# statgen/popscle

Measured on AMD Instinct MI355X. Metric: cell-sample-pair LLs/sec (singlet+doublet), demuxlet 10k cells×16 samples, higher is better.
Workload: dtype f64; 1 GPU; demuxlet synthetic PLP (BASELINE.json configs[1]): 10000 cells x 16 samples x 50000 SNPs per GPU, alpha grid [0.0, 0.5], 9537271 entries, 12399525 reads; cells_per_gpu=10000, samples=16, snps=50000, entries_per_gpu=9537271, lls_per_cell=256, parallelism=cells sharded x1

## Files before the change

### popscle_amd/csrc/demux_oct.hip

```cpp
#include <algorithm>
#include <vector>

#include <rocprim/device/device_radix_sort.hpp>

#include "demux_call_body.hpp"

namespace {

constexpr int O_NLUT = 129;
constexpr int O_LPAD = 3;

template <int P>
struct og {
  static_assert(P == 8 || P == 16, "eight or sixteen lanes per entry");
  static constexpr int SLOTS = 64 / P;
  static constexpr int BATCH = P;
  static constexpr int NROT = P / 2 - 1;
  static constexpr int N_ACC = 3 + 4 * NROT + 3;
  static constexpr int N_HYP = N_ACC * P;
  static constexpr int SLOT_STRIDE = 9 * P + 2;
  static constexpr int ACC_AB = 2;
  static constexpr int ACC_F_AB = 3 + 4 * NROT, ACC_F_AA = ACC_F_AB + 1, ACC_F_BB = ACC_F_AB + 2;
  __host__ __device__ static constexpr int acc_single(int c) { return c; }
  __host__ __device__ static constexpr int acc_rot(int t, int c, int d) { return 3 + (t - 1) * 4 + c * 2 + d; }
  __host__ __device__ static constexpr int ror(int t) { return 0x120 + (P == 8 ? 2 * t : t); }
  __device__ static __forceinline__ int pos(int lane) { return P == 8 ? (lane >> 1) & 7 : lane & 15; }
  __device__ static __forceinline__ int slot(int lane) { return P == 8 ? ((lane >> 4) << 1) | (lane & 1) : lane >> 4; }
  __device__ static __forceinline__ int lane0(int lane) { return P == 8 ? lane & ~14 : lane & ~15; }
  static constexpr uint32_t MROW = 32u * P;
  static constexpr int TROW = 6 * P;
};

template <int CTRL>
__device__ __forceinline__ double dpp_rot(double x) {
  int lo = __double2loint(x), hi = __double2hiint(x);
  lo = __builtin_amdgcn_mov_dpp(lo, CTRL, 0xF, 0xF, false);
  hi = __builtin_amdgcn_mov_dpp(hi, CTRL, 0xF, 0xF, false);
  return __hiloint2double(hi, lo);
}

template <int P>
__global__ void oct_pmap_kernel(int32_t* pmap) {
  const int lane = threadIdx.x;
  const int p = og<P>::pos(lane);
  wave_for<1, P / 2 + 1>([&](auto tc) {
    constexpr int t = decltype(tc)::value;
    const int pt = __builtin_amdgcn_mov_dpp(p, og<P>::ror(t), 0xF, 0xF, false);
    if (og<P>::slot(lane) == 0) pmap[(t - 1) * P + p] = pt;
  });
}

__global__ void __launch_bounds__(64)
    oct_partition_kernel(int n_chunks, const row_chunk* __restrict__ chunks, const quad_entry* __restrict__ qent,
                         const uint32_t* __restrict__ lin, const uint8_t* __restrict__ reads,
                         const double* __restrict__ gp0s, quad_entry* __restrict__ out, quad_lrec* __restrict__ lrec,
                         int32_t* __restrict__ nlin) {
  const int q = blockIdx.x * blockDim.x + threadIdx.x;
  if (q >= n_chunks) return;
  const int64_t e0 = chunks[q].e0;
  const int len = chunks[q].len;
  int w = 0;
  for (int i = 0; i < len; ++i) {
    const int64_t e = e0 + i;
    if ((lin[e >> 5] >> (e & 31)) & 1u) {
      const quad_entry p = qent[e];
      uint32_t code = MUXGL_READ_OTHER;
      for (uint32_t k = 0; k < p.nreads; ++k) {
        const uint32_t bb = k < 4 ? (p.first4 >> (8 * k)) & 0xffu : (uint32_t)reads[(int64_t)p.r0 + k];
        if (bb != MUXGL_READ_OTHER) code = bb;
      }
      if (gp0s[p.snp] < 0.0) code = MUXGL_READ_OTHER;
      lrec[e0 + w] = quad_lrec{p.snp, code};
      out[e0 + w++] = p;
    }
  }
  nlin[q] = w;
  for (int i = 0; i < len; ++i) {
    const int64_t e = e0 + i;
    if (!((lin[e >> 5] >> (e & 31)) & 1u)) out[e0 + w++] = qent[e];
  }
}

constexpr int QUAD_BUCKET = 1024;
__global__ void __launch_bounds__(256)
    quad_order_key_kernel(int n_chunks, int bucket, const row_chunk* __restrict__ chunks,
                          const int32_t* __restrict__ chunk_nlin, uint64_t* __restrict__ key, int32_t* __restrict__ iota) {
  const int w = blockIdx.x * blockDim.x + threadIdx.x;
  if (w >= n_chunks) return;
  const int nl = chunk_nlin[w], len = chunks[w].len;
  const uint64_t bg = (uint64_t)min(len - nl, 1023), bl = (uint64_t)min(nl, 1023);
  key[w] = ((uint64_t)(w / bucket) << 40) | ((1023u - bg) << 30) | ((1023u - bl) << 20) | (uint64_t)(w % bucket);
  iota[w] = w;
}

__global__ void __launch_bounds__(256)
    oct_unit_steps_kernel(int n_units, int n_chunks, int slots, const int32_t* __restrict__ order,
                          const int32_t* __restrict__ nlin, int32_t* __restrict__ steps) {
  const int u = blockIdx.x * blockDim.x + threadIdx.x;
  if (u >= n_units) return;
  int m = 0;
  for (int k = 0; k < slots; ++k) {
    const int w = u * slots + k;
    if (w < n_chunks) m = max(m, nlin[order[w]]);
  }
  steps[u] = m > 0 ? (m + 2) / 3 * 3 + O_LPAD : 0;
}

__global__ void __launch_bounds__(256)
    oct_repack_kernel(int n_units, int n_chunks, const row_chunk* __restrict__ chunks, const int32_t* __restrict__ order,
                      const int32_t* __restrict__ nlin, const quad_lrec* __restrict__ lrec,
                      const int32_t* __restrict__ steps, const int64_t* __restrict__ unit_ptr, uint32_t S_dummy,
                      int slots, uint32_t mrow , uint2* __restrict__ orec) {
  const int t = blockIdx.x * blockDim.x + threadIdx.x;
  const int u = t / slots, slot = t % slots;
  if (u >= n_units) return;
  const int w = u * slots + slot;
  int64_t e0 = 0;
  int nl = 0;
  if (w < n_chunks) {
    const int q = order[w];
    e0 = chunks[q].e0;
    nl = nlin[q];
  }
  uint2* dst = orec + unit_ptr[u] + slot;
  const int n = steps[u];
  for (int i = 0; i < n; ++i) {
    uint2 r{S_dummy * mrow, (uint32_t)(O_NLUT - 1) * 32u};
    if (i < nl) {
      const quad_lrec x = lrec[e0 + i];
      const uint32_t idx = x.code == MUXGL_READ_OTHER ? (uint32_t)(O_NLUT - 1) : ((x.code >> 7) << 6) | (x.code & 0x3fu);
      r = uint2{(uint32_t)x.snp * mrow, idx * 32u};
    }
    dst[(size_t)i * slots] = r;
  }
}

template <int P, bool UNIT_S>
#ifndef OCT_WAVES
#define OCT_WAVES 3
#endif
__global__ void __launch_bounds__(64, P == 8 ? OCT_WAVES : 2)
    demux_oct_kernel(const row_chunk* __restrict__ chunks, int n_chunks, const quad_entry* __restrict__ qent,
                     const uint2* __restrict__ orec, const int64_t* __restrict__ unit_ptr,
                     const int32_t* __restrict__ chunk_nlin,
                     const int32_t* __restrict__ order, const uint8_t* __restrict__ reads,
                     const double* __restrict__ gpo, const double* __restrict__ gmo,
                     const double* __restrict__ gp0s, int32_t S_dummy, const double* __restrict__ lut_g,
                     const int32_t* __restrict__ chunk_pos, double* __restrict__ part_m, int32_t* __restrict__ part_e) {
  __shared__ double lut[384];
  __shared__ __align__(16) double ablut[O_NLUT * 4];
  using G = og<P>;
  constexpr int ON_ACC = G::N_ACC, O_SLOTS = G::SLOTS, O_BATCH = G::BATCH, O_SLOT_STRIDE = G::SLOT_STRIDE;
  constexpr int O_ACC_AB = G::ACC_AB, O_ACC_F_AB = G::ACC_F_AB, O_ACC_F_AA = G::ACC_F_AA, O_ACC_F_BB = G::ACC_F_BB;
  __shared__ __align__(16) double pgs[O_SLOTS * O_SLOT_STRIDE];
  __shared__ int32_t snps[64], snps_nx[64];

  const int lane = threadIdx.x;
  const int p = G::pos(lane);
  const int slot = G::slot(lane);
  for (int i = lane; i < 384; i += 64) lut[i] = lut_g[i];
  for (int i = lane; i < O_NLUT; i += 64) {
    const uint32_t bq = (uint32_t)i & 0x3f;
    const bool ref = (i >> 6) == 0;
    const double e3 = lut_g[256 + bq], mt = lut_g[128 + bq];
    const double pR = ref ? mt : e3, pA = ref ? e3 : mt;
    const double mx = fmax(pR, pA);
    double x = __builtin_amdgcn_rcp(mx);
    x = fma(x, fma(-mx, x, 1.0), x);
    x = fma(x, fma(-mx, x, 1.0), x);
    const double cc = 1.0 / (1.0 + 1e-10);
    const double sc = cc * x, tt = 1e-10 * cc;
    const bool none = i == O_NLUT - 1;
    const double B = none ? 0.0 : (pA - pR) * (0.25 * sc);
    ablut[4 * i] = none ? 1.0 : fma(pR, sc, tt);
    ablut[4 * i + 1] = B;
    ablut[4 * i + 2] = B + B;
    ablut[4 * i + 3] = 0.0;
  }
  __syncthreads();

  const int unit = xcd_swizzle(blockIdx.x, gridDim.x >> 3);
  const int wq = unit * O_SLOTS + slot;
  const uint32_t p16 = (uint32_t)p * 16u;
  const int q = wq < n_chunks ? (order ? order[wq] : wq) : n_chunks;
  int64_t e0 = 0;
  int len = 0;
  int32_t qpos = 0;
  if (q < n_chunks) {
    e0 = chunks[q].e0;
    len = chunks[q].len;
    qpos = chunk_pos[q];
  }
  const int nl = (chunk_nlin && q < n_chunks) ? chunk_nlin[q] : 0;
  const int nLmax = wave_max_i32(nl);
  const int ngmax = wave_max_i32(len - nl);
  const int nb = (ngmax + O_BATCH - 1) / O_BATCH;

  double acc[ON_ACC];
  int32_t exs[ON_ACC];
#pragma unroll
  for (int a = 0; a < ON_ACC; ++a) {
    acc[a] = 1.0;
    exs[a] = 0;
  }
  double accW[2] = {1.0, 1.0};
  int32_t exW[2] = {0, 0};
  double accH = 1.0;
  int32_t exH = 0;

  auto renorm = [&]() __attribute__((always_inline)) {
#pragma unroll
    for (int a = 0; a < ON_ACC; ++a) prodacc_renorm(acc[a], exs[a]);
    prodacc_renorm(accW[0], exW[0]);
    prodacc_renorm(accW[1], exW[1]);
    prodacc_renorm(accH, exH);
  };

  if (nLmax > 0) {
    struct rowl_t {
      double sa, ra, sb, rb;
    };
    auto load_rowl = [&](rowl_t& R, uint32_t row_off) __attribute__((always_inline)) {
      if (UNIT_S) {
        const double2 v = *reinterpret_cast<const double2*>(reinterpret_cast<const char*>(gmo) + (size_t)((row_off >> 1) + p16));
        R.sa = R.sb = 1.0;
        R.ra = v.x;
        R.rb = v.y;
        return;
      }
      const double2* pc = reinterpret_cast<const double2*>(reinterpret_cast<const char*>(gmo) + (size_t)(row_off + p16));
      const double2 va = pc[0], vb = pc[P];
      R.sa = va.x;
      R.ra = va.y;
      R.sb = vb.x;
      R.rb = vb.y;
    };
    const uint2* lr = orec + unit_ptr[unit] + slot;
    struct ab_t {
      double A, B, B2;
    };
    auto ab_of = [&](const uint2& rc) __attribute__((always_inline)) {
      const double* t = reinterpret_cast<const double*>(reinterpret_cast<const char*>(ablut) + rc.y);
      const double2 v = *reinterpret_cast<const double2*>(t);
      return ab_t{v.x, v.y, t[2]};
    };
    auto sweepL = [&](const rowl_t& R, const ab_t& ab) __attribute__((always_inline)) {
      const double A = ab.A, B = ab.B, B2 = ab.B2;
      if (!UNIT_S) {
        accW[0] *= R.sa;
        accW[1] *= R.sb;
      }
      acc[G::acc_single(0)] *= fma(B2, R.ra, A);
      acc[G::acc_single(1)] *= fma(B2, R.rb, A);
      const double Xa = fma(B, R.ra, A), Xb = fma(B, R.rb, A);
      acc[O_ACC_AB] *= fma(B, R.rb, Xa);
      wave_for<1, G::NROT + 1>([&](auto tc) {
        constexpr int t = decltype(tc)::value;
        const double Pa = dpp_rot<G::ror(t)>(R.ra), Pb = dpp_rot<G::ror(t)>(R.rb);
        acc[G::acc_rot(t, 0, 0)] *= fma(B, Pa, Xa);
        acc[G::acc_rot(t, 0, 1)] *= fma(B, Pb, Xa);
        acc[G::acc_rot(t, 1, 0)] *= fma(B, Pa, Xb);
        acc[G::acc_rot(t, 1, 1)] *= fma(B, Pb, Xb);
      });
      {
        const double Pa = dpp_rot<G::ror(P / 2)>(R.ra), Pb = dpp_rot<G::ror(P / 2)>(R.rb);
        acc[O_ACC_F_AB] *= fma(B, Pb, Xa);
        acc[O_ACC_F_AA] *= fma(B, Pa, Xa);
        acc[O_ACC_F_BB] *= fma(B, Pb, Xb);
      }
    };
    auto step = [&](int i, const rowl_t& Rc, rowl_t& Rnn, const ab_t& abc, ab_t& abn, uint2& rc0, const uint2& rc1,
                    const uint2& rc2) __attribute__((always_inline)) {
      rc0 = lr[(i + 3) * O_SLOTS];
      abn = ab_of(rc1);
      load_rowl(Rnn, rc2.x);
      __builtin_amdgcn_sched_barrier(0);
      sweepL(Rc, abc);
      __builtin_amdgcn_sched_barrier(0);
    };
    rowl_t L0, L1, L2;
    ab_t ab0, ab1, ab2;
    uint2 ra = lr[0], rb = lr[O_SLOTS], rc = lr[2 * O_SLOTS];
    load_rowl(L0, ra.x);
    load_rowl(L1, rb.x);
    ab0 = ab_of(ra);
    int since = 0;
    for (int i = 0; i < nLmax; i += 3) {
      step(i, L0, L2, ab0, ab1, ra, rb, rc);
      step(i + 1, L1, L0, ab1, ab2, rb, rc, ra);
      step(i + 2, L2, L1, ab2, ab0, rc, ra, rb);
      if (++since == 10) {
        since = 0;
        renorm();
      }
    }
    renorm();
  }

  if (nb > 0) {
    const int last = len > 0 ? len - 1 : 0;
    auto fetch_meta = [&](int b) __attribute__((always_inline)) {
      const int idx = nl + b * O_BATCH + p;
      return qent[e0 + (idx < last ? idx : last)];
    };
    auto snp_of = [&](const quad_entry& r, int b) __attribute__((always_inline)) { return (nl + b * O_BATCH + p < len) ? r.snp : -1; };
    quad_entry precA = fetch_meta(0), precB = fetch_meta(1);
    double hs_cur = gp0s[precA.snp];

    struct row_t {
      double a[3], b[3];
    };
    auto load_row = [&](row_t& R, int32_t s) __attribute__((always_inline)) {
      const double2* pc = reinterpret_cast<const double2*>(gpo + (size_t)s * G::TROW) + p;
      const double2 v0 = pc[0], v1 = pc[P], v2 = pc[2 * P];
      R.a[0] = v0.x;
      R.a[1] = v0.y;
      R.a[2] = v1.x;
      R.b[0] = v1.y;
      R.b[1] = v2.x;
      R.b[2] = v2.y;
    };

    auto phase1 = [&](int b) __attribute__((always_inline)) {
      const int32_t sa = snp_of(precA, b);
      const int32_t s = (hs_cur >= 0.0) ? sa : -1;
      const double hs_out = (s >= 0) ? hs_cur : 1.0;
      const int64_t r0 = precA.r0, r1 = (int64_t)precA.r0 + precA.nreads;
      const uint32_t first4 = precA.first4;
      precA = precB;
      precB = fetch_meta(b + 2);
      hs_cur = gp0s[precA.snp];
      double q0[3], q1[5];
      {
        double pRk[4], pAk[4];
        const uint32_t nr = (s >= 0) ? (uint32_t)(r1 - r0) : 0u;
#pragma unroll
        for (int k = 0; k < 4; ++k) {
          const uint32_t bb = (first4 >> (8 * k)) & 0xffu;
          const uint32_t bq = bb & 0x7f;
          const double e3 = lut[256 + bq], mt = lut[128 + bq];
          const bool use = (uint32_t)k < nr && bb != MUXGL_READ_OTHER;
          const bool ref = (bb >> 7) == 0;
          pRk[k] = use ? (ref ? mt : e3) : 1.0;
          pAk[k] = use ? (ref ? e3 : mt) : 1.0;
        }
        {
          const double d = pAk[0] - pRk[0];
          const double mid = fma(d, 0.5, pRk[0]);
          q0[0] = pRk[0];
          q0[1] = mid;
          q0[2] = pAk[0];
          q1[0] = pRk[0];
          q1[1] = fma(d, 0.25, pRk[0]);
          q1[2] = mid;
          q1[3] = fma(d, 0.75, pRk[0]);
          q1[4] = pAk[0];
        }
#pragma unroll
        for (int k = 1; k < 4; ++k) {
          const double d = pAk[k] - pRk[k];
          const double mid = fma(d, 0.5, pRk[k]);
          q0[0] *= pRk[k];
          q0[1] *= mid;
          q0[2] *= pAk[k];
          q1[0] *= pRk[k];
          q1[1] *= fma(d, 0.25, pRk[k]);
          q1[2] *= mid;
          q1[3] *= fma(d, 0.75, pRk[k]);
          q1[4] *= pAk[k];
        }
        if (nr > 4) {
          int since = 4;
          for (int64_t rr = r0 + 4; rr < r1; ++rr) {
            const uint32_t bb = (uint32_t)reads[rr];
            if (bb == MUXGL_READ_OTHER) continue;
            const uint32_t al = bb >> 7, bq = bb & 0x7f;
            const double e3 = lut[256 + bq], mt = lut[128 + bq];
            const double pR = (al == 0) ? mt : e3, pA = (al == 0) ? e3 : mt;
            const double d = pA - pR;
            const double mid = fma(d, 0.5, pR);
            q0[0] *= pR;
            q0[1] *= mid;
            q0[2] *= pA;
            q1[0] *= pR;
            q1[1] *= fma(d, 0.25, pR);
            q1[2] *= mid;
            q1[3] *= fma(d, 0.75, pR);
            q1[4] *= pA;
            if (++since >= 32) {
              since = 0;
              double mx = fmax(fmax(q0[0], q0[1]), q0[2]);
#pragma unroll
              for (int t = 0; t < 5; ++t) mx = fmax(mx, q1[t]);
              const double inv = 1.0 / mx;
#pragma unroll
              for (int l = 0; l < 3; ++l) q0[l] *= inv;
#pragma unroll
              for (int t = 0; t < 5; ++t) q1[t] *= inv;
            }
          }
        }
        double mx = fmax(fmax(q0[0], q0[1]), q0[2]);
#pragma unroll
        for (int t = 0; t < 5; ++t) mx = fmax(mx, q1[t]);
        double x = __builtin_amdgcn_rcp(mx);
        x = fma(x, fma(-mx, x, 1.0), x);
        x = fma(x, fma(-mx, x, 1.0), x);
        const double cc = 1.0 / (1.0 + 1e-10);
        const double sc = (s >= 0) ? cc * x : 1.0, tt = (s >= 0) ? 1e-10 * cc : 0.0;
#pragma unroll
        for (int l = 0; l < 3; ++l) q0[l] = fma(q0[l], sc, tt);
#pragma unroll
        for (int t = 0; t < 5; ++t) q1[t] = fma(q1[t], sc, tt);
      }
      double* dst = pgs + slot * O_SLOT_STRIDE + p * 8;
      dst[0] = q0[0];
      dst[1] = q0[1];
      dst[2] = q0[2];
#pragma unroll
      for (int t = 0; t < 5; ++t) dst[3 + t] = q1[t];
      pgs[slot * O_SLOT_STRIDE + 8 * P + p] = hs_out;
      snps[slot * P + p] = (s >= 0) ? s : S_dummy;
      const int32_t sn = snp_of(precA, b + 1);
      snps_nx[slot * P + p] = (sn >= 0) ? sn : S_dummy;
    };

    auto sweep_entry = [&](const row_t& R, int i) __attribute__((always_inline)) {
      const double* qq = pgs + slot * O_SLOT_STRIDE + i * 8;
      const double a0 = qq[0], a1 = qq[1], a2 = qq[2];
      const double b0 = qq[3], b1 = qq[4], b2 = qq[5], b3 = qq[6], b4 = qq[7];
      if (!UNIT_S) accH *= pgs[slot * O_SLOT_STRIDE + 8 * P + i];
      acc[G::acc_single(0)] *= fma(R.a[2], a2, fma(R.a[1], a1, R.a[0] * a0));
      acc[G::acc_single(1)] *= fma(R.b[2], a2, fma(R.b[1], a1, R.b[0] * a0));
      double ua[3], ub[3];
      ua[0] = fma(R.a[2], b2, fma(R.a[1], b1, R.a[0] * b0));
      ua[1] = fma(R.a[2], b3, fma(R.a[1], b2, R.a[0] * b1));
      ua[2] = fma(R.a[2], b4, fma(R.a[1], b3, R.a[0] * b2));
      ub[0] = fma(R.b[2], b2, fma(R.b[1], b1, R.b[0] * b0));
      ub[1] = fma(R.b[2], b3, fma(R.b[1], b2, R.b[0] * b1));
      ub[2] = fma(R.b[2], b4, fma(R.b[1], b3, R.b[0] * b2));
      auto dot = [](const double* g, const double* u) { return fma(g[2], u[2], fma(g[1], u[1], g[0] * u[0])); };
      acc[O_ACC_AB] *= dot(R.b, ua);
      wave_for<1, G::NROT + 1>([&](auto tc) {
        constexpr int t = decltype(tc)::value;
        double Pa[3], Pb[3];
        Pa[0] = dpp_rot<G::ror(t)>(R.a[0]);
        Pa[1] = dpp_rot<G::ror(t)>(R.a[1]);
        Pa[2] = dpp_rot<G::ror(t)>(R.a[2]);
        Pb[0] = dpp_rot<G::ror(t)>(R.b[0]);
        Pb[1] = dpp_rot<G::ror(t)>(R.b[1]);
        Pb[2] = dpp_rot<G::ror(t)>(R.b[2]);
        acc[G::acc_rot(t, 0, 0)] *= dot(Pa, ua);
        acc[G::acc_rot(t, 0, 1)] *= dot(Pb, ua);
        acc[G::acc_rot(t, 1, 0)] *= dot(Pa, ub);
        acc[G::acc_rot(t, 1, 1)] *= dot(Pb, ub);
      });
      {
        constexpr int CF = G::ror(P / 2);
        double Pa[3], Pb[3];
        Pa[0] = dpp_rot<CF>(R.a[0]);
        Pa[1] = dpp_rot<CF>(R.a[1]);
        Pa[2] = dpp_rot<CF>(R.a[2]);
        Pb[0] = dpp_rot<CF>(R.b[0]);
        Pb[1] = dpp_rot<CF>(R.b[1]);
        Pb[2] = dpp_rot<CF>(R.b[2]);
        acc[O_ACC_F_AB] *= dot(Pb, ua);
        acc[O_ACC_F_AA] *= dot(Pa, ua);
        acc[O_ACC_F_BB] *= dot(Pb, ub);
      }
    };

    auto batch = [&](int b, row_t& X, row_t& Y, row_t& Z) __attribute__((always_inline)) {
      phase1(b);
      __syncthreads();
      const int32_t* sn = snps + slot * P;
      const int32_t* sx = snps_nx + slot * P;
      const int lim = (b == nb - 1) ? ngmax - b * O_BATCH : O_BATCH;
      auto set = [&](auto ic) __attribute__((always_inline)) -> row_t& {
        constexpr int i = decltype(ic)::value % 3;
        if constexpr (i == 0) return X;
        else if constexpr (i == 1) return Y;
        else return Z;
      };
      bool go = true;
      wave_for<0, P>([&](auto ec) {
        constexpr int e = decltype(ec)::value;
        if (!go) return;
        load_row(set(std::integral_constant<int, e + 2>{}), e + 2 < P ? sn[e + 2 < P ? e + 2 : 0] : sx[e + 2 - P < 0 ? 0 : e + 2 - P]);
        __builtin_amdgcn_sched_barrier(0);
        sweep_entry(set(ec), e);
        __builtin_amdgcn_sched_barrier(0);
        if (lim <= e + 1) go = false;
      });
      if (P == 16 || (b & 1)) renorm();
      __syncthreads();
    };

    row_t R0, R1, R2;
    snps_nx[slot * P + p] = (snp_of(precA, 0) >= 0) ? precA.snp : S_dummy;
    __syncthreads();
    load_row(R0, snps_nx[slot * P + 0]);
    load_row(R1, snps_nx[slot * P + 1]);
    __syncthreads();
    for (int b = 0; b < nb; b += 3) {
      batch(b, R0, R1, R2);
      if (b + 1 >= nb) break;
      if (P == 8) batch(b + 1, R2, R0, R1);
      else batch(b + 1, R1, R2, R0);
      if (b + 2 >= nb) break;
      if (P == 8) batch(b + 2, R1, R2, R0);
      else batch(b + 2, R2, R0, R1);
    }
    renorm();
  }

  {
    int32_t exa[ON_ACC];
    const double wa = accW[0], wb = accW[1];
    const int32_t ea = exW[0], eb = exW[1];
    const int src0 = G::lane0(lane);
    const double W0 = __shfl(wa, src0, 64) * accH;
    const int32_t e0w = __shfl(ea, src0, 64) + exH;
    acc[G::acc_single(0)] *= wa * W0;
    exa[G::acc_single(0)] = ea + e0w;
    acc[G::acc_single(1)] *= wb * W0;
    exa[G::acc_single(1)] = eb + e0w;
    acc[O_ACC_AB] *= wa * wb;
    exa[O_ACC_AB] = ea + eb;
    wave_for<1, G::NROT + 1>([&](auto tc) {
      constexpr int T = decltype(tc)::value, CTRL = G::ror(T);
      const double pa = dpp_rot<CTRL>(wa), pb = dpp_rot<CTRL>(wb);
      const int32_t qa = __builtin_amdgcn_mov_dpp(ea, CTRL, 0xF, 0xF, false);
      const int32_t qb = __builtin_amdgcn_mov_dpp(eb, CTRL, 0xF, 0xF, false);
      acc[G::acc_rot(T, 0, 0)] *= wa * pa;
      exa[G::acc_rot(T, 0, 0)] = ea + qa;
      acc[G::acc_rot(T, 0, 1)] *= wa * pb;
      exa[G::acc_rot(T, 0, 1)] = ea + qb;
      acc[G::acc_rot(T, 1, 0)] *= wb * pa;
      exa[G::acc_rot(T, 1, 0)] = eb + qa;
      acc[G::acc_rot(T, 1, 1)] *= wb * pb;
      exa[G::acc_rot(T, 1, 1)] = eb + qb;
    });
    {
      constexpr int CF = G::ror(P / 2);
      const double pa = dpp_rot<CF>(wa), pb = dpp_rot<CF>(wb);
      const int32_t qa = __builtin_amdgcn_mov_dpp(ea, CF, 0xF, 0xF, false);
      const int32_t qb = __builtin_amdgcn_mov_dpp(eb, CF, 0xF, 0xF, false);
      acc[O_ACC_F_AB] *= wa * pb;
      exa[O_ACC_F_AB] = ea + qb;
      acc[O_ACC_F_AA] *= wa * pa;
      exa[O_ACC_F_AA] = ea + qa;
      acc[O_ACC_F_BB] *= wb * pb;
      exa[O_ACC_F_BB] = eb + qb;
    }
    if (q < n_chunks) {
#pragma unroll
      for (int a = 0; a < ON_ACC; ++a) {
        int e;
        const double m = frexp(acc[a], &e);
        part_m[((size_t)qpos * ON_ACC + a) * P + p] = m;
        part_e[((size_t)qpos * ON_ACC + a) * P + p] = exs[a] + e + exa[a];
      }
    }
  }
}

template <int P>
__device__ __forceinline__ bool oct_decode(int idx, const int32_t* __restrict__ pmap, int V, int& j, int& k) {
  using G = og<P>;
  const int a = idx / P, p = idx % P;
  bool publish = true;
  if (a < 2) {
    j = p + P * a;
    k = 0;
  } else if (a == G::ACC_AB) {
    j = p + P;
    k = p;
  } else if (a < G::ACC_F_AB) {
    const int t = (a - 3) >> 2, c = ((a - 3) >> 1) & 1, d = (a - 3) & 1;
    j = p + P * c;
    k = pmap[t * P + p] + P * d;
  } else {
    const int pf = pmap[G::NROT * P + p];
    if (a == G::ACC_F_AB) {
      j = p;
      k = pf + P;
    } else if (a == G::ACC_F_AA) {
      j = p;
      k = pf;
      publish = p < pf;
    } else {
      j = p + P;
      k = pf + P;
      publish = p < pf;
    }
  }
  return publish && j < V && k < V;
}

__device__ __forceinline__ double oct_log(double m, int64_t e) { return pos_log(m, (double)e); }

template <int P>
__device__ __forceinline__ bool oct_hypothesis(int idx, int64_t c0, int64_t c1, const double* __restrict__ part_m,
                                               const int32_t* __restrict__ part_e, const int32_t* __restrict__ pmap, int V,
                                               int& j, int& k, double& v) {
  constexpr int O_NHYP = og<P>::N_HYP;
  if (!oct_decode<P>(idx, pmap, V, j, k)) return false;
  double m = 1.0;
  int64_t e = 0;
  int cnt = 0;
  for (int64_t ci = c0; ci < c1; ci += 8) {
    double pm[8];
    int32_t pe[8];
#pragma unroll
    for (int u = 0; u < 8; ++u) {
      const bool ok = ci + u < c1;
      const size_t o = (size_t)(ok ? ci + u : c0) * O_NHYP + idx;
      pm[u] = ok ? part_m[o] : 1.0;
      pe[u] = ok ? part_e[o] : 0;
    }
#pragma unroll
    for (int u = 0; u < 8; ++u) {
      m *= pm[u];
      e += pe[u];
    }
    if (++cnt == 64) {
      cnt = 0;
      int ee;
      m = frexp(m, &ee);
      e += ee;
    }
  }
  v = oct_log(m, e);
  return true;
}

__global__ void __launch_bounds__(256)
    oct_chunk_pos_kernel(int64_t n_chunks, const int32_t* __restrict__ cell_chunks, int32_t* __restrict__ pos) {
  const int64_t ci = (int64_t)blockIdx.x * blockDim.x + threadIdx.x;
  if (ci < n_chunks) pos[cell_chunks[ci]] = (int32_t)ci;
}

template <int P>
__global__ void __launch_bounds__(192)
    demux_oct_reduce_kernel(const int64_t* __restrict__ cell_chunk_ptr, const double* __restrict__ part_m,
                            const int32_t* __restrict__ part_e, const int32_t* __restrict__ pmap, int V,
                            double* __restrict__ ll) {
  const int64_t c = blockIdx.x;
  const int64_t c0 = cell_chunk_ptr[c], c1 = cell_chunk_ptr[c + 1];
  if (c0 == c1) return;
  double* out = ll + (size_t)c * V * V * 2;
  for (int idx = threadIdx.x; idx < og<P>::N_HYP; idx += 192) {
    int j, k;
    double v;
    if (!oct_hypothesis<P>(idx, c0, c1, part_m, part_e, pmap, V, j, k, v)) continue;
    if (idx < 2 * P) {
      out[((size_t)j * V + k) * 2 + 0] = v;
    } else {
      out[((size_t)j * V + k) * 2 + 1] = v;
      out[((size_t)k * V + j) * 2 + 1] = v;
    }
  }
}

#ifndef QF_CELLS_N
#define QF_CELLS_N 4
#endif
template <int P>
__global__ void __launch_bounds__(256)
    demux_oct_finish_kernel(int64_t C, const int64_t* __restrict__ cell_ptr, const int64_t* __restrict__ cell_chunk_ptr,
                            const double* __restrict__ part_m, const int32_t* __restrict__ part_e,
                            const int32_t* __restrict__ pmap, int V,
                            muxgl_call::call_alpha al, double doublet_prior, muxgl_demux_cell* __restrict__ out) {
  constexpr int QF_CELLS = P == 8 ? QF_CELLS_N : 1, THREADS = 256, O_NHYP = og<P>::N_HYP;
  static_assert(P == 16 || QF_CELLS * 64 == THREADS, "a wave per cell at P = 8");
  constexpr int LD = 4 * P + 1;
  __shared__ double llt[QF_CELLS][2 * P * LD];
  __shared__ __align__(16) muxgl_demux_cell rec[QF_CELLS];
  __shared__ int64_t ccp[QF_CELLS + 1];
  static_assert(sizeof(muxgl_demux_cell) % 16 == 0, "records are copied out in 16-byte pieces");
  const int64_t cbase = (int64_t)blockIdx.x * QF_CELLS;
  const int tid = threadIdx.x;
  if (tid <= QF_CELLS) ccp[tid] = cell_chunk_ptr[cbase + tid <= C ? cbase + tid : C];
  for (int t = tid; t < QF_CELLS * 2 * P * LD; t += THREADS) (&llt[0][0])[t] = 0.0;
  __syncthreads();
  constexpr int NH = (QF_CELLS * O_NHYP + THREADS - 1) / THREADS;
  int hj[NH], hk[NH], hidx[NH], hlc[NH];
  int64_t h0[NH];
  int hn[NH];
  bool hv[NH];
  double hm[NH];
  int64_t he[NH];
  int nmax = 0;
#pragma unroll
  for (int i = 0; i < NH; ++i) {
    const int w = tid + i * THREADS;
    const int lc = w < QF_CELLS * O_NHYP ? w / O_NHYP : 0;
    hlc[i] = lc;
    hidx[i] = w - lc * O_NHYP;
    h0[i] = ccp[lc];
    hn[i] = (int)(ccp[lc + 1] - ccp[lc]);
    hv[i] = w < QF_CELLS * O_NHYP && hn[i] > 0 && oct_decode<P>(hidx[i] < O_NHYP ? hidx[i] : 0, pmap, V, hj[i], hk[i]);
    if (!hv[i]) hn[i] = 0, hidx[i] = 0;
    hm[i] = 1.0;
    he[i] = 0;
    nmax = hn[i] > nmax ? hn[i] : nmax;
  }
  int cnt = 0;
  for (int ci = 0; ci < nmax; ci += 4) {
    double pm[NH][4];
    int32_t pe[NH][4];
#pragma unroll
    for (int i = 0; i < NH; ++i)
#pragma unroll
      for (int u = 0; u < 4; ++u) {
        const bool ok = ci + u < hn[i];
        const size_t o = (ok ? (size_t)(h0[i] + ci + u) * O_NHYP : 0) + hidx[i];
        const double vm = part_m[o];
        const int32_t ve = part_e[o];
        pm[i][u] = ok ? vm : 1.0;
        pe[i][u] = ok ? ve : 0;
      }
#pragma unroll
    for (int i = 0; i < NH; ++i)
#pragma unroll
      for (int u = 0; u < 4; ++u) {
        hm[i] *= pm[i][u];
        he[i] += pe[i][u];
      }
    if (++cnt == 128) {
      cnt = 0;
#pragma unroll
      for (int i = 0; i < NH; ++i) {
        int ee;
        hm[i] = frexp(hm[i], &ee);
        he[i] += ee;
      }
    }
  }
#pragma unroll
  for (int i = 0; i < NH; ++i) {
    if (!hv[i]) continue;
    const double v = oct_log(hm[i], he[i]);
    if (hidx[i] < 2 * P) {
      llt[hlc[i]][hj[i] * LD + hk[i] * 2 + 0] = v;
    } else {
      llt[hlc[i]][hj[i] * LD + hk[i] * 2 + 1] = v;
      llt[hlc[i]][hk[i] * LD + hj[i] * 2 + 1] = v;
    }
  }
  __syncthreads();
  if constexpr (P == 8) {
    __shared__ muxgl_call::call_partial parts[QF_CELLS];
    const int lc = tid >> 6;
    const int64_t c = cbase + lc;
    const muxgl_call::call_partial cp = muxgl_call::demux_call_scan<16, 4>(tid & 63, c < C, V, 2, al, llt[lc], LD);
    if ((tid & 63) == 0) parts[lc] = cp;
    __syncthreads();
    if (tid < QF_CELLS && cbase + tid < C)
      muxgl_call::demux_call_decide(parts[tid], (int32_t)(cell_ptr[cbase + tid + 1] - cell_ptr[cbase + tid]), V, 2, al,
                                    &rec[tid]);
  } else {
    if (tid < 64)
      muxgl_call::demux_call_group<64>(tid, cbase < C, cbase < C ? (int32_t)(cell_ptr[cbase + 1] - cell_ptr[cbase]) : 0, V, 2,
                                       al, doublet_prior, llt[0], &rec[0], LD);
  }
  __syncthreads();
  constexpr int NQ = (int)(sizeof(muxgl_demux_cell) / 16);
  if (tid < QF_CELLS * NQ && cbase + tid / NQ < C)
    reinterpret_cast<uint4*>(out + cbase)[tid] = reinterpret_cast<const uint4*>(&rec[0])[tid];
}

}

int quad_launch_order(muxgl_handle* h, const row_chunk* d_chunks, const int32_t* d_nlin, int64_t n, int32_t** order) {
  int32_t* d_iota = nullptr;
  uint64_t *d_key = nullptr, *d_key2 = nullptr;
  void* d_tmp = nullptr;
  auto cleanup = [&]() {
    dev_free(&d_iota);
    dev_free(&d_key);
    dev_free(&d_key2);
    if (d_tmp) (void)hipFree(d_tmp);
    d_tmp = nullptr;
  };
  if (dev_alloc(h, order, (size_t)n) || dev_alloc(h, &d_iota, (size_t)n) || dev_alloc(h, &d_key, (size_t)n) ||
      dev_alloc(h, &d_key2, (size_t)n)) {
    cleanup();
    return 1;
  }
  int bucket = QUAD_BUCKET;
  if (const char* ev = getenv("MUXGL_QUAD_BUCKET")) bucket = atoi(ev) > 0 ? atoi(ev) : bucket;
  if (bucket > (1 << 20)) bucket = 1 << 20;
  hipLaunchKernelGGL(quad_order_key_kernel, dim3((unsigned)((n + 255) / 256)), dim3(256), 0, h->stream, (int)n, bucket, d_chunks,
                     d_nlin, d_key, d_iota);
  size_t tmp_bytes = 0;
  hipError_t e = rocprim::radix_sort_pairs(nullptr, tmp_bytes, d_key, d_key2, d_iota, *order, (size_t)n, 0u, 64u, h->stream);
  if (e == hipSuccess) e = dev_malloc_retry((void**)&d_tmp, tmp_bytes ? tmp_bytes : 1);
  if (e == hipSuccess) e = rocprim::radix_sort_pairs(d_tmp, tmp_bytes, d_key, d_key2, d_iota, *order, (size_t)n, 0u, 64u, h->stream);
  if (e == hipSuccess) e = hipStreamSynchronize(h->stream);
  cleanup();
  if (e != hipSuccess) MUXGL_FAIL(h, "quad_launch_order: %s", hipGetErrorString(e));
  return 0;
}

namespace {
template <int P>
int oct_launch_t(muxgl_handle* h, const muxgl_demux_params* p) {
  constexpr int O_SLOTS = og<P>::SLOTS, O_NHYP = og<P>::N_HYP;
  muxgl_row_state* st = h->qrow;
  if (!st->d_tmap || st->tmap_p != P) {
    if (dev_alloc(h, &st->d_tmap, (size_t)(P / 2) * P)) return 1;
    hipLaunchKernelGGL(oct_pmap_kernel<P>, dim3(1), dim3(64), 0, h->stream, st->d_tmap);
    HIPCHK(h, hipGetLastError());
    st->tmap_p = P;
  }
  const size_t need = (size_t)st->n_chunks * O_NHYP;
  if (need > st->part_cap) {
    if (dev_alloc(h, &st->d_part, need)) return 1;
    st->part_cap = need;
  }
  if (need > st->part_e_cap) {
    if (dev_alloc(h, &st->d_part_e, need)) return 1;
    st->part_e_cap = need;
  }
  if (!st->d_chunk_pos) {
    if (dev_alloc(h, &st->d_chunk_pos, (size_t)(st->n_chunks ? st->n_chunks : 1))) return 1;
    if (st->n_chunks)
      hipLaunchKernelGGL(oct_chunk_pos_kernel, dim3((unsigned)((st->n_chunks + 255) / 256)), dim3(256), 0, h->stream, st->n_chunks,
                         st->d_cell_chunks, st->d_chunk_pos);
    HIPCHK(h, hipGetLastError());
  }
  const bool use_lin = h->d_lin && h->d_gmq && !(h->flags & MUXGL_FLAG_NO_LINEAR_ENTRIES);
  const unsigned blocks = (unsigned)((((st->n_chunks + O_SLOTS - 1) / O_SLOTS) + 7) / 8 * 8);
  if (use_lin && !st->d_chunk_nlin && st->n_chunks) {
    quad_lrec* d_lrec = nullptr;
    int32_t* d_steps = nullptr;
    auto cleanup = [&]() {
      dev_free(&d_lrec);
      dev_free(&d_steps);
    };
    if (dev_alloc(h, &st->d_qent_lin, (size_t)h->nnz) || dev_alloc(h, &st->d_chunk_nlin, (size_t)st->n_chunks) ||
        dev_alloc(h, &d_lrec, (size_t)h->nnz)) {
      cleanup();
      return 1;
    }
    hipLaunchKernelGGL(oct_partition_kernel, dim3((unsigned)((st->n_chunks + 63) / 64)), dim3(64), 0, h->stream,
                       (int)st->n_chunks, st->d_chunks, h->d_qent, h->d_lin, h->d_reads, h->d_gp0s, st->d_qent_lin,
                       d_lrec, st->d_chunk_nlin);
    if (hipGetLastError() != hipSuccess || quad_launch_order(h, st->d_chunks, st->d_chunk_nlin, st->n_chunks, &st->d_quad_order)) {
      cleanup();
      MUXGL_FAIL(h, "demux_oct_launch: partition failed");
    }
    const int n_units = (int)blocks;
    std::vector<int32_t> steps((size_t)n_units);
    std::vector<int64_t> uptr((size_t)n_units + 1, 0);
    if (dev_alloc(h, &d_steps, (size_t)n_units)) {
      cleanup();
      return 1;
    }
    hipLaunchKernelGGL(oct_unit_steps_kernel, dim3((unsigned)((n_units + 255) / 256)), dim3(256), 0, h->stream, n_units,
                       (int)st->n_chunks, O_SLOTS, st->d_quad_order, st->d_chunk_nlin, d_steps);
    hipError_t e = hipMemcpyAsync(steps.data(), d_steps, sizeof(int32_t) * (size_t)n_units, hipMemcpyDeviceToHost, h->stream);
    if (e == hipSuccess) e = hipStreamSynchronize(h->stream);
    for (int u = 0; u < n_units; ++u) uptr[(size_t)u + 1] = uptr[(size_t)u] + (int64_t)steps[(size_t)u] * O_SLOTS;
    if (e != hipSuccess || dev_alloc(h, &st->d_unit_ptr, uptr.size()) || dev_alloc(h, &st->d_orec, (size_t)uptr.back() + 1)) {
      cleanup();
      MUXGL_FAIL(h, "demux_oct_launch: record tables");
    }
    e = hipMemcpyAsync(st->d_unit_ptr, uptr.data(), sizeof(int64_t) * uptr.size(), hipMemcpyHostToDevice, h->stream);
    hipLaunchKernelGGL(oct_repack_kernel, dim3((unsigned)(((size_t)n_units * O_SLOTS + 255) / 256)), dim3(256), 0, h->stream,
                       n_units, (int)st->n_chunks, st->d_chunks, st->d_quad_order, st->d_chunk_nlin, d_lrec, d_steps,
                       st->d_unit_ptr, (uint32_t)h->S, O_SLOTS, og<P>::MROW, st->d_orec);
    if (e == hipSuccess) e = hipGetLastError();
    if (e == hipSuccess) e = hipStreamSynchronize(h->stream);
    cleanup();
    if (e != hipSuccess) MUXGL_FAIL(h, "demux_oct_launch: %s", hipGetErrorString(e));
  }
  tic(h, MUXGL_T_DEMUX_SWEEP);
  if (blocks) {
    auto kern = h->gp_unit_sums ? demux_oct_kernel<P, true> : demux_oct_kernel<P, false>;
    hipLaunchKernelGGL(kern, dim3(blocks), dim3(64), 0,
                       h->stream, st->d_chunks, (int)st->n_chunks,
                       use_lin ? st->d_qent_lin : h->d_qent, st->d_orec, st->d_unit_ptr,
                       use_lin ? st->d_chunk_nlin : (const int32_t*)nullptr,
                       use_lin ? st->d_quad_order : (const int32_t*)nullptr, h->d_reads,
                       h->d_gpq, h->d_gmq, h->d_gp0s, (int32_t)h->S, h->d_lut, st->d_chunk_pos, st->d_part, st->d_part_e);
    HIPCHK(h, hipGetLastError());
  }
  toc_tic(h, MUXGL_T_DEMUX_SWEEP, MUXGL_T_DEMUX_REDUCE);
  if (h->want_full_ll) {
    hipLaunchKernelGGL(demux_oct_reduce_kernel<P>, dim3((unsigned)h->C), dim3(192), 0, h->stream, st->d_cell_chunk_ptr,
                       st->d_part, st->d_part_e, st->d_tmap, h->V, h->d_ll);
  } else {
    const muxgl_call::call_alpha al = muxgl_call::make_call_alpha(p, h->V);
    constexpr int QF_CELLS = P == 8 ? QF_CELLS_N : 1;
    hipLaunchKernelGGL(demux_oct_finish_kernel<P>, dim3((unsigned)((h->C + QF_CELLS - 1) / QF_CELLS)), dim3(256), 0,
                       h->stream, h->C, h->d_cell_ptr, st->d_cell_chunk_ptr, st->d_part, st->d_part_e, st->d_tmap, h->V, al,
                       p->doublet_prior, h->h_dcells);
    h->records_on_host = true;
  }
  HIPCHK(h, hipGetLastError());
  toc(h, MUXGL_T_DEMUX_REDUCE);
  return 0;
}
}

int demux_oct_launch(muxgl_handle* h, const muxgl_demux_params* p) {
  return h->V <= 16 ? oct_launch_t<8>(h, p) : oct_launch_t<16>(h, p);
}
```

Before: 7.647 billion LLs/s.

## Pack partial mantissa and exponent into one 8-byte word with escape side channel

The sweep kernel now stores each partial product as a single 8-byte word: 52 mantissa bits plus a biased 12-bit exponent. A separate int32 side array is written only when the value falls outside the normal range. The reduce and finish kernels read one word per partial instead of a double plus an int32, and use a precomputed slot table for hypothesis decode. The finish kernel also now gives each cell its own wave with no per-hypothesis length masking. This is meant to cut memory traffic and per-element work in the reduction, at the cost of extra bit manipulation and a rare slow escape path.

```diff
diff --git a/popscle_amd/csrc/demux_oct.hip b/popscle_amd/csrc/demux_oct.hip
--- a/popscle_amd/csrc/demux_oct.hip
+++ b/popscle_amd/csrc/demux_oct.hip
@@ -31,6 +31,25 @@
   static constexpr int TROW = 6 * P;
 };
 
+constexpr int OCT_EBIAS = 4093;
+constexpr uint32_t OCT_EFIELD_ESC = 4095u;
+__device__ __forceinline__ void oct_pack(double m, int32_t E, size_t o, uint2* __restrict__ part, int32_t* __restrict__ part_e) {
+  const uint32_t hi = (uint32_t)__double2hiint(m), lo = (uint32_t)__double2loint(m);
+  const bool plain = (hi >> 20) == 0x3FEu && (uint32_t)(E + OCT_EBIAS) < OCT_EFIELD_ESC;
+  part[o] = uint2{lo, (hi & 0xFFFFFu) | ((plain ? (uint32_t)(E + OCT_EBIAS) : OCT_EFIELD_ESC) << 20)};
+  if (!plain) part_e[o] = (int32_t)(((uint32_t)E & 0xFFFFFu) | ((hi >> 20) << 20));
+}
+__device__ __forceinline__ void oct_unpack(uint2 w, size_t o, const int32_t* __restrict__ part_e, double& m, int32_t& eb) {
+  uint32_t top = 0x3FEu;
+  eb = (int32_t)(w.y >> 20);
+  if (w.y >= (OCT_EFIELD_ESC << 20)) {
+    const int32_t pe = part_e[o];
+    top = (uint32_t)pe >> 20;
+    eb = ((int32_t)((uint32_t)pe << 12) >> 12) + OCT_EBIAS;
+  }
+  m = __hiloint2double((int)((w.y & 0xFFFFFu) | (top << 20)), (int)w.x);
+}
+
 template <int CTRL>
 __device__ __forceinline__ double dpp_rot(double x) {
   int lo = __double2loint(x), hi = __double2hiint(x);
@@ -146,7 +165,7 @@
                      const int32_t* __restrict__ order, const uint8_t* __restrict__ reads,
                      const double* __restrict__ gpo, const double* __restrict__ gmo,
                      const double* __restrict__ gp0s, int32_t S_dummy, const double* __restrict__ lut_g,
-                     const int32_t* __restrict__ chunk_pos, double* __restrict__ part_m, int32_t* __restrict__ part_e) {
+                     const int32_t* __restrict__ chunk_pos, uint2* __restrict__ part, int32_t* __restrict__ part_e) {
   __shared__ double lut[384];
   __shared__ __align__(16) double ablut[O_NLUT * 4];
   using G = og<P>;
@@ -558,15 +577,14 @@
       for (int a = 0; a < ON_ACC; ++a) {
         int e;
         const double m = frexp(acc[a], &e);
-        part_m[((size_t)qpos * ON_ACC + a) * P + p] = m;
-        part_e[((size_t)qpos * ON_ACC + a) * P + p] = exs[a] + e + exa[a];
+        oct_pack(m, exs[a] + e + exa[a], ((size_t)qpos * ON_ACC + a) * P + p, part, part_e);
       }
     }
   }
 }
 
 template <int P>
-__device__ __forceinline__ bool oct_decode(int idx, const int32_t* __restrict__ pmap, int V, int& j, int& k) {
+__device__ __forceinline__ bool oct_decode(int idx, const int32_t* __restrict__ pmap, int& j, int& k) {
   using G = og<P>;
   const int a = idx / P, p = idx % P;
   bool publish = true;
@@ -595,44 +613,80 @@
       publish = p < pf;
     }
   }
-  return publish && j < V && k < V;
-}
+  return publish;
+}
+
+template <int P>
+__global__ void __launch_bounds__(64) oct_slot_kernel(const int32_t* __restrict__ pmap, int32_t* __restrict__ slots) {
+  const int idx = blockIdx.x * blockDim.x + threadIdx.x;
+  if (idx >= og<P>::N_HYP) return;
+  int j, k;
+  const bool publish = oct_decode<P>(idx, pmap, j, k);
+  slots[idx] = j | (k << 8) | ((publish ? (j > k ? j : k) : 255) << 16);
+}
+constexpr int32_t OCT_SLOT_NONE = 255 << 16;
+__device__ __forceinline__ bool oct_slot_live(int32_t s, int V) { return ((s >> 16) & 0xff) < V; }
 
 __device__ __forceinline__ double oct_log(double m, int64_t e) { return pos_log(m, (double)e); }
 
-template <int P>
-__device__ __forceinline__ bool oct_hypothesis(int idx, int64_t c0, int64_t c1, const double* __restrict__ part_m,
-                                               const int32_t* __restrict__ part_e, const int32_t* __restrict__ pmap, int V,
-                                               int& j, int& k, double& v) {
-  constexpr int O_NHYP = og<P>::N_HYP;
-  if (!oct_decode<P>(idx, pmap, V, j, k)) return false;
-  double m = 1.0;
-  int64_t e = 0;
+template <int NH, int U, int O_NHYP, int R>
+__device__ __forceinline__ void oct_fold_trip(const uint2* __restrict__ pb, const int32_t* __restrict__ pe, int64_t ci,
+                                              const int (&off)[NH], double (&hm)[NH], int64_t (&he)[NH]) {
+  uint2 w[NH][R];
+  uint32_t top = 0;
+#pragma unroll
+  for (int i = 0; i < NH; ++i)
+#pragma unroll
+    for (int u = 0; u < R; ++u) {
+      w[i][u] = pb[(size_t)(ci + u) * O_NHYP + off[i]];
+      top = w[i][u].y > top ? w[i][u].y : top;
+    }
+  if (__builtin_expect(top < (OCT_EFIELD_ESC << 20), 1)) {
+#pragma unroll
+    for (int i = 0; i < NH; ++i) {
+      uint32_t es = 0;
+#pragma unroll
+      for (int u = 0; u < R; ++u) {
+        hm[i] *= __hiloint2double((int)((w[i][u].y & 0xFFFFFu) | 0x3FE00000u), (int)w[i][u].x);
+        es += w[i][u].y >> 20;
+      }
+      he[i] += es;
+    }
+  } else {
+#pragma unroll
+    for (int i = 0; i < NH; ++i)
+#pragma unroll
+      for (int u = 0; u < R; ++u) {
+        double m;
+        int32_t eb;
+        oct_unpack(w[i][u], (size_t)(ci + u) * O_NHYP + off[i], pe, m, eb);
+        hm[i] *= m;
+        he[i] += eb;
+      }
+  }
+}
+template <int NH, int U, int O_NHYP>
+__device__ __forceinline__ void oct_fold(const uint2* __restrict__ pb, const int32_t* __restrict__ pe, int64_t n,
+                                         const int (&off)[NH], double (&hm)[NH], int64_t (&he)[NH]) {
+  static_assert(U == 4 || U == 8, "the last trip is spelled per remainder");
+  int64_t ci = 0;
   int cnt = 0;
-  for (int64_t ci = c0; ci < c1; ci += 8) {
-    double pm[8];
-    int32_t pe[8];
-#pragma unroll
-    for (int u = 0; u < 8; ++u) {
-      const bool ok = ci + u < c1;
-      const size_t o = (size_t)(ok ? ci + u : c0) * O_NHYP + idx;
-      pm[u] = ok ? part_m[o] : 1.0;
-      pe[u] = ok ? part_e[o] : 0;
-    }
-#pragma unroll
-    for (int u = 0; u < 8; ++u) {
-      m *= pm[u];
-      e += pe[u];
-    }
-    if (++cnt == 64) {
+  for (; ci + U <= n; ci += U) {
+    oct_fold_trip<NH, U, O_NHYP, U>(pb, pe, ci, off, hm, he);
+    if (++cnt == 512 / U) {
       cnt = 0;
-      int ee;
-      m = frexp(m, &ee);
-      e += ee;
-    }
-  }
-  v = oct_log(m, e);
-  return true;
+#pragma unroll
+      for (int i = 0; i < NH; ++i) {
+        int ee;
+        hm[i] = frexp(hm[i], &ee);
+        he[i] += ee;
+      }
+    }
+  }
+  wave_for<1, U>([&](auto rc) {
+    constexpr int R = decltype(rc)::value;
+    if (n - ci == R) oct_fold_trip<NH, U, O_NHYP, R>(pb, pe, ci, off, hm, he);
+  });
 }
 
 __global__ void __launch_bounds__(256)
@@ -643,18 +697,33 @@
 
 template <int P>
 __global__ void __launch_bounds__(192)
-    demux_oct_reduce_kernel(const int64_t* __restrict__ cell_chunk_ptr, const double* __restrict__ part_m,
-                            const int32_t* __restrict__ part_e, const int32_t* __restrict__ pmap, int V,
+    demux_oct_reduce_kernel(const int64_t* __restrict__ cell_chunk_ptr, const uint2* __restrict__ part,
+                            const int32_t* __restrict__ part_e, const int32_t* __restrict__ slots, int V,
                             double* __restrict__ ll) {
+  constexpr int O_NHYP = og<P>::N_HYP, NH = (O_NHYP + 191) / 192;
   const int64_t c = blockIdx.x;
   const int64_t c0 = cell_chunk_ptr[c], c1 = cell_chunk_ptr[c + 1];
   if (c0 == c1) return;
   double* out = ll + (size_t)c * V * V * 2;
-  for (int idx = threadIdx.x; idx < og<P>::N_HYP; idx += 192) {
-    int j, k;
-    double v;
-    if (!oct_hypothesis<P>(idx, c0, c1, part_m, part_e, pmap, V, j, k, v)) continue;
-    if (idx < 2 * P) {
+  int32_t hs[NH];
+  int off[NH];
+  double hm[NH];
+  int64_t he[NH];
+#pragma unroll
+  for (int i = 0; i < NH; ++i) {
+    const int idx = (int)threadIdx.x + i * 192;
+    hs[i] = idx < O_NHYP ? slots[idx] : OCT_SLOT_NONE;
+    off[i] = oct_slot_live(hs[i], V) ? idx : 0;
+    hm[i] = 1.0;
+    he[i] = 0;
+  }
+  oct_fold<NH, 8, O_NHYP>(part + (size_t)c0 * O_NHYP, part_e + (size_t)c0 * O_NHYP, c1 - c0, off, hm, he);
+#pragma unroll
+  for (int i = 0; i < NH; ++i) {
+    if (!oct_slot_live(hs[i], V)) continue;
+    const int j = hs[i] & 0xff, k = (hs[i] >> 8) & 0xff;
+    const double v = oct_log(hm[i], he[i] - (int64_t)OCT_EBIAS * (c1 - c0));
+    if (i == 0 && (int)threadIdx.x < 2 * P) {
       out[((size_t)j * V + k) * 2 + 0] = v;
     } else {
       out[((size_t)j * V + k) * 2 + 1] = v;
@@ -663,97 +732,61 @@
   }
 }
 
-#ifndef QF_CELLS_N
-#define QF_CELLS_N 4
-#endif
 template <int P>
 __global__ void __launch_bounds__(256)
     demux_oct_finish_kernel(int64_t C, const int64_t* __restrict__ cell_ptr, const int64_t* __restrict__ cell_chunk_ptr,
-                            const double* __restrict__ part_m, const int32_t* __restrict__ part_e,
-                            const int32_t* __restrict__ pmap, int V,
+                            const uint2* __restrict__ part, const int32_t* __restrict__ part_e,
+                            const int32_t* __restrict__ slots, int V,
                             muxgl_call::call_alpha al, double doublet_prior, muxgl_demux_cell* __restrict__ out) {
-  constexpr int QF_CELLS = P == 8 ? QF_CELLS_N : 1, THREADS = 256, O_NHYP = og<P>::N_HYP;
-  static_assert(P == 16 || QF_CELLS * 64 == THREADS, "a wave per cell at P = 8");
+  constexpr int THREADS = 256, TC = P == 8 ? 64 : 256, QF_CELLS = THREADS / TC, O_NHYP = og<P>::N_HYP;
   constexpr int LD = 4 * P + 1;
   __shared__ double llt[QF_CELLS][2 * P * LD];
   __shared__ __align__(16) muxgl_demux_cell rec[QF_CELLS];
-  __shared__ int64_t ccp[QF_CELLS + 1];
   static_assert(sizeof(muxgl_demux_cell) % 16 == 0, "records are copied out in 16-byte pieces");
-  const int64_t cbase = (int64_t)blockIdx.x * QF_CELLS;
   const int tid = threadIdx.x;
-  if (tid <= QF_CELLS) ccp[tid] = cell_chunk_ptr[cbase + tid <= C ? cbase + tid : C];
-  for (int t = tid; t < QF_CELLS * 2 * P * LD; t += THREADS) (&llt[0][0])[t] = 0.0;
-  __syncthreads();
-  constexpr int NH = (QF_CELLS * O_NHYP + THREADS - 1) / THREADS;
-  int hj[NH], hk[NH], hidx[NH], hlc[NH];
-  int64_t h0[NH];
-  int hn[NH];
+  const int lc = __builtin_amdgcn_readfirstlane(tid / TC), t = tid % TC;
+  constexpr int NH = (O_NHYP + TC - 1) / TC;
+  int off[NH], at[NH], atm[NH];
   bool hv[NH];
-  double hm[NH];
-  int64_t he[NH];
-  int nmax = 0;
 #pragma unroll
   for (int i = 0; i < NH; ++i) {
-    const int w = tid + i * THREADS;
-    const int lc = w < QF_CELLS * O_NHYP ? w / O_NHYP : 0;
-    hlc[i] = lc;
-    hidx[i] = w - lc * O_NHYP;
-    h0[i] = ccp[lc];
-    hn[i] = (int)(ccp[lc + 1] - ccp[lc]);
-    hv[i] = w < QF_CELLS * O_NHYP && hn[i] > 0 && oct_decode<P>(hidx[i] < O_NHYP ? hidx[i] : 0, pmap, V, hj[i], hk[i]);
-    if (!hv[i]) hn[i] = 0, hidx[i] = 0;
-    hm[i] = 1.0;
-    he[i] = 0;
-    nmax = hn[i] > nmax ? hn[i] : nmax;
-  }
-  int cnt = 0;
-  for (int ci = 0; ci < nmax; ci += 4) {
-    double pm[NH][4];
-    int32_t pe[NH][4];
-#pragma unroll
-    for (int i = 0; i < NH; ++i)
-#pragma unroll
-      for (int u = 0; u < 4; ++u) {
-        const bool ok = ci + u < hn[i];
-        const size_t o = (ok ? (size_t)(h0[i] + ci + u) * O_NHYP : 0) + hidx[i];
-        const double vm = part_m[o];
-        const int32_t ve = part_e[o];
-        pm[i][u] = ok ? vm : 1.0;
-        pe[i][u] = ok ? ve : 0;
-      }
-#pragma unroll
-    for (int i = 0; i < NH; ++i)
-#pragma unroll
-      for (int u = 0; u < 4; ++u) {
-        hm[i] *= pm[i][u];
-        he[i] += pe[i][u];
-      }
-    if (++cnt == 128) {
-      cnt = 0;
-#pragma unroll
-      for (int i = 0; i < NH; ++i) {
-        int ee;
-        hm[i] = frexp(hm[i], &ee);
-        he[i] += ee;
-      }
-    }
-  }
-#pragma unroll
-  for (int i = 0; i < NH; ++i) {
-    if (!hv[i]) continue;
-    const double v = oct_log(hm[i], he[i]);
-    if (hidx[i] < 2 * P) {
-      llt[hlc[i]][hj[i] * LD + hk[i] * 2 + 0] = v;
-    } else {
-      llt[hlc[i]][hj[i] * LD + hk[i] * 2 + 1] = v;
-      llt[hlc[i]][hk[i] * LD + hj[i] * 2 + 1] = v;
-    }
+    const int idx = t + i * TC;
+    const int32_t s = idx < O_NHYP ? slots[idx] : OCT_SLOT_NONE;
+    const int j = s & 0xff, k = (s >> 8) & 0xff;
+    hv[i] = oct_slot_live(s, V);
+    off[i] = hv[i] ? idx : 0;
+    const bool single = i == 0 && t < 2 * P;
+    at[i] = j * LD + k * 2 + (single ? 0 : 1);
+    atm[i] = single ? at[i] : k * LD + j * 2 + 1;
+  }
+  const int64_t cbase = (int64_t)blockIdx.x * QF_CELLS, c = cbase + lc;
+  int64_t c0 = 0, n = 0;
+  if (c < C) {
+    c0 = cell_chunk_ptr[c];
+    n = cell_chunk_ptr[c + 1] - c0;
+  }
+  if (n > 0) {
+    double hm[NH];
+    int64_t he[NH];
+#pragma unroll
+    for (int i = 0; i < NH; ++i) {
+      hm[i] = 1.0;
+      he[i] = 0;
+    }
+    oct_fold<NH, 4, O_NHYP>(part + (size_t)c0 * O_NHYP, part_e + (size_t)c0 * O_NHYP, n, off, hm, he);
+#pragma unroll
+    for (int i = 0; i < NH; ++i) {
+      if (!hv[i]) continue;
+      const double v = oct_log(hm[i], he[i] - (int64_t)OCT_EBIAS * n);
+      llt[lc][at[i]] = v;
+      llt[lc][atm[i]] = v;
+    }
+  } else {
+    for (int x = t; x < 2 * P * LD; x += TC) llt[lc][x] = 0.0;
   }
   __syncthreads();
   if constexpr (P == 8) {
     __shared__ muxgl_call::call_partial parts[QF_CELLS];
-    const int lc = tid >> 6;
-    const int64_t c = cbase + lc;
     const muxgl_call::call_partial cp = muxgl_call::demux_call_scan<16, 4>(tid & 63, c < C, V, 2, al, llt[lc], LD);
     if ((tid & 63) == 0) parts[lc] = cp;
     __syncthreads();
@@ -809,12 +842,15 @@
 int oct_launch_t(muxgl_handle* h, const muxgl_demux_params* p) {
   constexpr int O_SLOTS = og<P>::SLOTS, O_NHYP = og<P>::N_HYP;
   muxgl_row_state* st = h->qrow;
+  constexpr int N_PMAP = (P / 2) * P;
   if (!st->d_tmap || st->tmap_p != P) {
-    if (dev_alloc(h, &st->d_tmap, (size_t)(P / 2) * P)) return 1;
+    if (dev_alloc(h, &st->d_tmap, (size_t)N_PMAP + O_NHYP)) return 1;
     hipLaunchKernelGGL(oct_pmap_kernel<P>, dim3(1), dim3(64), 0, h->stream, st->d_tmap);
+    hipLaunchKernelGGL(oct_slot_kernel<P>, dim3((O_NHYP + 63) / 64), dim3(64), 0, h->stream, st->d_tmap, st->d_tmap + N_PMAP);
     HIPCHK(h, hipGetLastError());
     st->tmap_p = P;
   }
+  const int32_t* d_slots = st->d_tmap + N_PMAP;
   const size_t need = (size_t)st->n_chunks * O_NHYP;
   if (need > st->part_cap) {
     if (dev_alloc(h, &st->d_part, need)) return 1;
@@ -824,6 +860,7 @@
     if (dev_alloc(h, &st->d_part_e, need)) return 1;
     st->part_e_cap = need;
   }
+  uint2* d_part = reinterpret_cast<uint2*>(st->d_part);
   if (!st->d_chunk_pos) {
     if (dev_alloc(h, &st->d_chunk_pos, (size_t)(st->n_chunks ? st->n_chunks : 1))) return 1;
     if (st->n_chunks)
@@ -885,19 +922,20 @@
                        use_lin ? st->d_qent_lin : h->d_qent, st->d_orec, st->d_unit_ptr,
                        use_lin ? st->d_chunk_nlin : (const int32_t*)nullptr,
                        use_lin ? st->d_quad_order : (const int32_t*)nullptr, h->d_reads,
-                       h->d_gpq, h->d_gmq, h->d_gp0s, (int32_t)h->S, h->d_lut, st->d_chunk_pos, st->d_part, st->d_part_e);
+                       h->d_gpq, h->d_gmq, h->d_gp0s, (int32_t)h->S, h->d_lut, st->d_chunk_pos, d_part, st->d_part_e);
     HIPCHK(h, hipGetLastError());
   }
   toc_tic(h, MUXGL_T_DEMUX_SWEEP, MUXGL_T_DEMUX_REDUCE);
   if (h->want_full_ll) {
     hipLaunchKernelGGL(demux_oct_reduce_kernel<P>, dim3((unsigned)h->C), dim3(192), 0, h->stream, st->d_cell_chunk_ptr,
-                       st->d_part, st->d_part_e, st->d_tmap, h->V, h->d_ll);
+                       d_part, st->d_part_e, d_slots, h->V, h->d_ll);
   } else {
     const muxgl_call::call_alpha al = muxgl_call::make_call_alpha(p, h->V);
-    constexpr int QF_CELLS = P == 8 ? QF_CELLS_N : 1;
-    hipLaunchKernelGGL(demux_oct_finish_kernel<P>, dim3((unsigned)((h->C + QF_CELLS - 1) / QF_CELLS)), dim3(256), 0,
-                       h->stream, h->C, h->d_cell_ptr, st->d_cell_chunk_ptr, st->d_part, st->d_part_e, st->d_tmap, h->V, al,
-                       p->doublet_prior, h->h_dcells);
+    constexpr int QF_CELLS = P == 8 ? 4 : 1;
+    const int64_t n_groups = (h->C + QF_CELLS - 1) / QF_CELLS;
+    if (n_groups)
+      hipLaunchKernelGGL(demux_oct_finish_kernel<P>, dim3((unsigned)n_groups), dim3(256), 0, h->stream, h->C, h->d_cell_ptr,
+                         st->d_cell_chunk_ptr, d_part, st->d_part_e, d_slots, h->V, al, p->doublet_prior, h->h_dcells);
     h->records_on_host = true;
   }
   HIPCHK(h, hipGetLastError());
```

After: 7.912 billion LLs/s (median of 6 runs). +3.5%, better.
